# zcablii/RS_detection

Hardware: NVIDIA B200
Metric: tiles/s (Oriented R-CNN rotated-box hot path: RoIAlignRotated fwd + obb2poly + per-class nms_rotated) (higher is better)
Workload: dtype f32

## Files before the change

### rs_detection_b200/csrc/nms.cu

```cuda
#include <cub/device/device_radix_sort.cuh>
#include <cub/device/device_scan.cuh>
#include <cub/device/device_select.cuh>
#include <thrust/iterator/counting_iterator.h>

#include <mutex>
#include <vector>

#include "common.cuh"
#include "nms_engine.cuh"
#include "poly_iou.cuh"
#include "rotated_iou.cuh"

namespace rsdet {

constexpr int kNmsThreads = 128;
constexpr int kReduceThreads = 256;
constexpr size_t kCubTempBytes = 8u << 20;
constexpr int kFastSegs = 2048;

struct HBox { double x1, y1, x2, y2; };

template <int KIND> struct Traits;

template <> struct Traits<RSDET_NMS_ROTATED> {
    using Box = RBox; using Raw = float; using Thr = float;
    static constexpr int kRow = 5; static constexpr bool kScratch = true;
    __device__ static Box prep(const Raw* r) { return prep_rbox(r, 0); }
    static constexpr bool kRefine = true;
    __device__ static bool cheap(const Box& a, const Box& b) { return rbox_may_overlap(a, b); }
    __device__ static bool refine1(const Box& a, const Box& b, Thr thr) { return !rbox_iou_below(a, b, thr); }
    __device__ static bool refine2(const Box& a, const Box& b, Thr thr) { return !rbox_iou_below_strips(a, b, thr); }
    __device__ static bool suppress(const Box& a, const Box& b, Thr thr, float2* q) {
        return rotated_iou_pair<kNmsThreads>(a, b, q) > thr;
    }
};
template <> struct Traits<RSDET_NMS_ROTATED_GE> : Traits<RSDET_NMS_ROTATED> {
    __device__ static bool suppress(const Box& a, const Box& b, Thr thr, float2* q) {
        return rotated_iou_pair<kNmsThreads>(a, b, q) >= thr;
    }
};
template <> struct Traits<RSDET_NMS_POLY> {
    using Box = PolyBox; using Raw = float; using Thr = float;
    static constexpr int kRow = 8; static constexpr bool kScratch = true;
    __device__ static Box prep(const Raw* r) { return prep_polybox(r); }
    static constexpr bool kRefine = false;
    __device__ static bool cheap(const Box& a, const Box& b) { return !poly_pair_is_zero(a, b); }
    __device__ static bool refine1(const Box&, const Box&, Thr) { return true; }
    __device__ static bool refine2(const Box&, const Box&, Thr) { return true; }
    __device__ static bool suppress(const Box& a, const Box& b, Thr thr, float2* q) {
        return poly_iou_f32<kNmsThreads>(a, b, q) > thr;
    }
};
template <> struct Traits<RSDET_NMS_MERGE> {
    using Box = MBox; using Raw = double; using Thr = double;
    static constexpr int kRow = 8; static constexpr bool kScratch = false;
    __device__ static Box prep(const Raw* r) {
        Box b;
        double x1 = r[0], x2 = r[0], y1 = r[1], y2 = r[1];
        for (int i = 0; i < 4; i++) {
            b.p[2 * i] = r[2 * i]; b.p[2 * i + 1] = r[2 * i + 1];
            x1 = fmin(x1, r[2 * i]); x2 = fmax(x2, r[2 * i]);
            y1 = fmin(y1, r[2 * i + 1]); y2 = fmax(y2, r[2 * i + 1]);
        }
        b.x1 = x1; b.y1 = y1; b.x2 = x2; b.y2 = y2;
        return b;
    }
    static constexpr bool kRefine = false;
    __device__ static bool cheap(const Box& a, const Box& b) { return merge_hbb_overlap(a, b); }
    __device__ static bool refine1(const Box&, const Box&, Thr) { return true; }
    __device__ static bool refine2(const Box&, const Box&, Thr) { return true; }
    __device__ static bool suppress(const Box& a, const Box& b, Thr thr, float2*) { return !(iou_poly_d(a, b) <= thr); }
};
template <> struct Traits<RSDET_NMS_HBB> {
    using Box = HBox; using Raw = double; using Thr = double;
    static constexpr int kRow = 4; static constexpr bool kScratch = false;
    __device__ static Box prep(const Raw* r) { Box b; b.x1 = r[0]; b.y1 = r[1]; b.x2 = r[2]; b.y2 = r[3]; return b; }
    static constexpr bool kRefine = false;
    __device__ static bool cheap(const Box& a, const Box& b) {
        return (fmin(a.x2, b.x2) > fmax(a.x1, b.x1) && fmin(a.y2, b.y2) > fmax(a.y1, b.y1)) ||
               (a.x2 - a.x1) * (a.y2 - a.y1) + (b.x2 - b.x1) * (b.y2 - b.y1) == 0.0;
    }
    __device__ static bool refine1(const Box&, const Box&, Thr) { return true; }
// ... 540 lines not shown
    __shared__ int s_count3;
    const int tid = threadIdx.x, lane = tid & 31;
    const int T = (n + 63) >> 6;
    const int total = T * (T + 1) / 2;
    for (int u = blockIdx.x; u < total; u += gridDim.x) {
        if (only_flagged && !only_flagged[u]) continue;
        __syncthreads();
        int rb = (int)(((2.0 * T + 1.0) - sqrt((2.0 * T + 1.0) * (2.0 * T + 1.0) - 8.0 * (double)u)) * 0.5);
        rb = max(0, min(rb, T - 1));
        while (rb > 0 && rb * T - rb * (rb - 1) / 2 > u) rb--;
        while ((rb + 1) * T - (rb + 1) * rb / 2 <= u) rb++;
        const int cb = rb + (u - (rb * T - rb * (rb - 1) / 2));
        const int nr = min(64, n - rb * 64), nc = min(64, n - cb * 64);
        if (tid < 64) {
            float4 rc = make_float4(0.f, 0.f, -1e30f, 0.f);
            if (tid < nr) {
                const RBox bx = boxes[rb * 64 + tid];
                s_row[tid] = bx;
                rc = make_float4(bx.x, bx.y, bx.r, 0.f);
            }
            s_rowc[tid] = rc;
        } else if (tid - 64 < nc) {
            s_col[tid - 64] = boxes[cb * 64 + tid - 64];
        }
        __syncthreads();
        const bool diag = rb == cb;
        {
            const int c = tid & 63, rhalf = tid >> 6;
            unsigned hits = 0u;
            if (c < nc) {
                const float cx = s_col[c].x, cy = s_col[c].y, cr = s_col[c].r;
#pragma unroll 8
                for (int k = 0; k < 32; k++) {
                    const int r = 2 * k + rhalf;
                    const float4 rc = s_rowc[r];
                    const float rs = rc.z + cr, dx = rc.x - cx, dy = rc.y - cy;
                    const bool cand = (rs >= 0.f) && !(dx * dx + dy * dy > rs * rs) && (!diag || c > r);
                    hits |= (cand ? 1u : 0u) << k;
                }
            }
            const int mine = __popc(hits);
            int incl = mine;
#pragma unroll
            for (int o = 1; o < 32; o <<= 1) {
                const int y = __shfl_up_sync(0xffffffffu, incl, o);
                if (lane >= o) incl += y;
            }
            if (lane == 31) s_wsum[tid >> 5] = incl;
            __syncthreads();
            int pos = incl - mine;
            for (int w = 0; w < (tid >> 5); w++) pos += s_wsum[w];
            if (tid == kNmsThreads - 1) s_count = pos + mine;
            while (hits) {
                const int k = __ffs(hits) - 1;
                hits &= hits - 1;
                s_queue[pos++] = (unsigned short)(((2 * k + rhalf) << 6) | c);
            }
        }
        __syncthreads();
        const int cnt = s_count;
        for (int q0 = 0; q0 < cnt; q0 += kQ2) {
            const int n2 = compact_queue(s_queue + q0, min(kQ2, cnt - q0), s_queue2, &s_count2, s_wsum,
                                         [&](int p) { return !rbox_iou_below(s_row[p >> 6], s_col[p & 63], thr); });
            const int n3 = compact_queue(s_queue2, n2, s_queue3, &s_count3, s_wsum,
                                         [&](int p) { return !rbox_iou_below_strips(s_row[p >> 6], s_col[p & 63], thr); });
            for (int qi = tid; qi < n3; qi += kNmsThreads) {
                const int p = s_queue3[qi];
                const int r = p >> 6, c = p & 63;
                const int a = rb * 64 + r, b = cb * 64 + c;
                const float iou_ab = rotated_iou_pair<kNmsThreads>(s_row[r], s_col[c], s_pts + tid);
                const bool d_ab = GE ? iou_ab >= thr : iou_ab > thr;
                bool d_ba = d_ab;
                if (fabsf(iou_ab - thr) <= 1e-5f) {
                    const float iou_ba = rotated_iou_pair<kNmsThreads>(s_col[c], s_row[r], s_pts + tid);
                    d_ba = GE ? iou_ba >= thr : iou_ba > thr;
                }
                if (d_ab) atomicOr(&ov[(size_t)a * pitch + (b >> 6)], 1ull << (b & 63));
                if (d_ba) atomicOr(&ov[(size_t)b * pitch + (a >> 6)], 1ull << (a & 63));
            }
        }
    }
}

template <bool GE>
__global__ void __launch_bounds__(kNmsThreads, 8)
ov_filter_kernel(const RBox* __restrict__ boxes, int n, float thr, int2* __restrict__ pairs, unsigned int cap,
                 unsigned int* __restrict__ pair_count, uint8_t* __restrict__ tile_flags) {
    __shared__ RBox s_row[64];
    __shared__ RBox s_col[64];
    __shared__ unsigned short s_queue[64 * 64];
    constexpr int kQ2 = 1024;
    __shared__ unsigned short s_queue2[kQ2];
    __shared__ unsigned short s_queue3[kQ2];
    __shared__ unsigned int s_base;
    __shared__ float4 s_rowc[64];
    __shared__ int s_wsum[kNmsThreads / 32];
    __shared__ int s_count;
    __shared__ int s_count2;
    __shared__ int s_count3;
    const int tid = threadIdx.x, lane = tid & 31;
    const int T = (n + 63) >> 6;
    const int total = T * (T + 1) / 2;
    for (int u = blockIdx.x; u < total; u += gridDim.x) {
        __syncthreads();
        int rb = (int)(((2.0 * T + 1.0) - sqrt((2.0 * T + 1.0) * (2.0 * T + 1.0) - 8.0 * (double)u)) * 0.5);
        rb = max(0, min(rb, T - 1));
        while (rb > 0 && rb * T - rb * (rb - 1) / 2 > u) rb--;
        while ((rb + 1) * T - (rb + 1) * rb / 2 <= u) rb++;
        const int cb = rb + (u - (rb * T - rb * (rb - 1) / 2));
        const int nr = min(64, n - rb * 64), nc = min(64, n - cb * 64);
        if (tid < 64) {
            float4 rc = make_float4(0.f, 0.f, -1e30f, 0.f);
            if (tid < nr) {
                const RBox bx = boxes[rb * 64 + tid];
                s_row[tid] = bx;
                rc = make_float4(bx.x, bx.y, bx.r, 0.f);
            }
            s_rowc[tid] = rc;
        } else if (tid - 64 < nc) {
            s_col[tid - 64] = boxes[cb * 64 + tid - 64];
        }
        __syncthreads();
        const bool diag = rb == cb;
        {
            const int c = tid & 63, rhalf = tid >> 6;
            unsigned hits = 0u;
            if (c < nc) {
                const float cx = s_col[c].x, cy = s_col[c].y, cr = s_col[c].r;
#pragma unroll 8
                for (int k = 0; k < 32; k++) {
                    const int r = 2 * k + rhalf;
                    const float4 rc = s_rowc[r];
                    const float rs = rc.z + cr, dx = rc.x - cx, dy = rc.y - cy;
                    const bool cand = (rs >= 0.f) && !(dx * dx + dy * dy > rs * rs) && (!diag || c > r);
                    hits |= (cand ? 1u : 0u) << k;
                }
            }
            const int mine = __popc(hits);
            int incl = mine;
#pragma unroll
            for (int o = 1; o < 32; o <<= 1) {
                const int y = __shfl_up_sync(0xffffffffu, incl, o);
                if (lane >= o) incl += y;
            }
            if (lane == 31) s_wsum[tid >> 5] = incl;
            __syncthreads();
            int pos = incl - mine;
            for (int w = 0; w < (tid >> 5); w++) pos += s_wsum[w];
            if (tid == kNmsThreads - 1) s_count = pos + mine;
            while (hits) {
                const int k = __ffs(hits) - 1;
                hits &= hits - 1;
                s_queue[pos++] = (unsigned short)(((2 * k + rhalf) << 6) | c);
            }
        }
        __syncthreads();
        const int cnt = s_count;
        for (int q0 = 0; q0 < cnt; q0 += kQ2) {
            const int n2 = compact_queue(s_queue + q0, min(kQ2, cnt - q0), s_queue2, &s_count2, s_wsum,
                                         [&](int p) { return !rbox_iou_below(s_row[p >> 6], s_col[p & 63], thr); });
            const int n3 = compact_queue(s_queue2, n2, s_queue3, &s_count3, s_wsum,
                                         [&](int p) { return !rbox_iou_below_strips(s_row[p >> 6], s_col[p & 63], thr); });
            if (tid == 0) {
                const unsigned int base = n3 ? atomicAdd(pair_count, (unsigned int)n3) : 0u;
                if (n3 && base + (unsigned int)n3 > cap) { tile_flags[u] = 1; atomicAdd(pair_count + 1, 1u); }
                s_base = base;
            }
            __syncthreads();
            const unsigned int base = s_base;
            for (int qi = tid; qi < n3; qi += kNmsThreads) {
                if (base + (unsigned int)qi < cap) {
                    const int p = s_queue3[qi];
                    pairs[base + qi] = make_int2(rb * 64 + (p >> 6), cb * 64 + (p & 63));
                }
            }
            __syncthreads();
        }
    }
}

template <bool GE>
__global__ void __launch_bounds__(kNmsThreads, 8)
ov_clip_kernel(const RBox* __restrict__ boxes, const int2* __restrict__ pairs, unsigned int cap, const unsigned int* __restrict__ pair_count,
               float thr, unsigned long long* __restrict__ ov, int pitch) {
    __shared__ float2 s_pts[24 * kNmsThreads];
    const unsigned int count = min(*pair_count, cap);
    const int tid = threadIdx.x;
    for (unsigned int i = blockIdx.x * kNmsThreads + tid; i < count; i += gridDim.x * kNmsThreads) {
        const int2 pr = pairs[i];
        const RBox A = boxes[pr.x], B = boxes[pr.y];
        const float iou_ab = rotated_iou_pair<kNmsThreads>(A, B, s_pts + tid);
        const bool d_ab = GE ? iou_ab >= thr : iou_ab > thr;
        bool d_ba = d_ab;
        if (fabsf(iou_ab - thr) <= 1e-5f) {
            const float iou_ba = rotated_iou_pair<kNmsThreads>(B, A, s_pts + tid);
            d_ba = GE ? iou_ba >= thr : iou_ba > thr;
        }
        if (d_ab) atomicOr(&ov[(size_t)pr.x * pitch + (pr.y >> 6)], 1ull << (pr.y & 63));
        if (d_ba) atomicOr(&ov[(size_t)pr.y * pitch + (pr.x >> 6)], 1ull << (pr.x & 63));
    }
}

__global__ void __launch_bounds__(kReduceThreads, 1)
reduce_ov_kernel(SegTable tb, const int* __restrict__ idx_ls, int cand_per_box, const unsigned long long* __restrict__ ov,
                 int pitch, int n_boxes, uint8_t* __restrict__ keep_sorted) {
    extern __shared__ unsigned long long s_remv[];
    __shared__ int s_box2[2][64];
    __shared__ unsigned int s_diag32[128];
    __shared__ unsigned int s_rem32[2];
    __shared__ unsigned long long s_keep;
    const int tid = threadIdx.x, lane = tid & 31;
    const int nseg = tb.hdr[0];
    const int T = (n_boxes + 63) >> 6;
    for (int s = blockIdx.x; s < nseg; s += gridDim.x) {
        const int st = tb.seg_start[s];
        const int ns = tb.seg_start[s + 1] - st;
        const int nblk = (ns + 63) >> 6;
        __syncthreads();
        for (int j = tid; j < T; j += kReduceThreads) s_remv[j] = 0ull;
        for (int b = 0; b < nblk; b++) {
            const int nr = min(64, ns - b * 64);
            int* s_box = s_box2[b & 1];
            if (tid < 64) s_box[tid] = tid < nr ? idx_ls[st + b * 64 + tid] / cand_per_box : -1;
            __syncthreads();
            if (tid < 64) {
                const int a = s_box[tid];
                const bool rem = a < 0 || ((s_remv[a >> 6] >> (a & 63)) & 1ull);
                const unsigned m = __ballot_sync(0xffffffffu, rem);
                if (lane == 0) s_rem32[tid >> 5] = m;
            }
#pragma unroll 4
            for (int it = 0; it < 16; it++) {
                const int idx = it * kReduceThreads + tid;
                const int i = idx >> 6, j = idx & 63;
                bool bit = false;
                if (i < nr && j < nr && j > i) {
                    const int a = s_box[i], c = s_box[j];
                    bit = (ov[(size_t)a * pitch + (c >> 6)] >> (c & 63)) & 1ull;
                }
                const unsigned m = __ballot_sync(0xffffffffu, bit);
                if (lane == 0) s_diag32[idx >> 5] = m;
            }
            __syncthreads();
            if (tid == 0) {
                unsigned long long r = (unsigned long long)s_rem32[0] | ((unsigned long long)s_rem32[1] << 32), kb = 0ull;
#pragma unroll
                for (int i = 0; i < 64; i++) {
                    const bool alive = ((r >> i) & 1ull) == 0ull;
                    const unsigned long long d = (unsigned long long)s_diag32[2 * i] | ((unsigned long long)s_diag32[2 * i + 1] << 32);
                    kb |= alive ? (1ull << i) : 0ull;
                    r |= alive ? d : 0ull;
                }
                s_keep = kb;
            }
            __syncthreads();
            const unsigned long long kb = s_keep;
            if (tid < nr) keep_sorted[st + b * 64 + tid] = (uint8_t)((kb >> tid) & 1ull);
            if (kb && b + 1 < nblk) {
                const int jj = tid & 63, rg = tid >> 6;
// ... 635 lines not shown

constexpr int kMaxNmsBoxes = 1 << 18;

size_t nms_ws_bytes(int kind, int n, size_t mask_words) {
    size_t N = (size_t)(n > 0 ? n : 1);
    size_t b = 0;
    b += 2 * ws_bytes<unsigned long long>(N);
    b += 4 * ws_bytes<int>(N);
    b += 2 * ws_bytes<uint32_t>(N);
    b += align256(box_bytes(kind) * N);
    b += ws_bytes<int32_t>(N);
    b += ws_bytes<int>(64) + ws_bytes<int>(N + 2) + 2 * ws_bytes<long long>(N + 2) + ws_bytes<double>(N + 1);
    b += ws_bytes<unsigned long long>(mask_words ? mask_words : N * ((N + 63) / 64));
    b += 3 * ws_bytes<uint8_t>(N);
    b += 2 * ws_bytes<int64_t>(N);
    b += ws_bytes<int>(64) + ws_bytes<int>(kFastSegs);
    b += ws_bytes<unsigned long long>(2 * N / 64 + 8) + ws_bytes<int>(2 * N / 64 + 8);
    b += align256(kCubTempBytes + 16 * N);
    return b;
}

template <int KIND>
static void launch_kind(const NmsArgs& a, const int* idx, void* boxes, int32_t* label_sorted, SegTable tb,
                        unsigned long long* mask, cudaStream_t st, bool mask_phase, int* starts_unsorted, const int* gate = nullptr) {
    using Tr = Traits<KIND>;
    if (!mask_phase) {
        prep_sorted_kernel<KIND><<<ceil_div(a.n_max, 256), 256, 0, st>>>((const typename Tr::Raw*)a.dets, a.labels, idx, a.n_max,
                                                                        a.n_dev, (typename Tr::Box*)boxes, label_sorted,
                                                                        tb.hdr, starts_unsorted);
    } else {
        long long T = (a.n_max + 63) / 64;
        long long tiles = T * (T + 1) / 2;
        int grid = (int)(tiles < (long long)kNumSMs * 5 ? tiles : (long long)kNumSMs * 5);
        mask_tiles_kernel<KIND><<<grid, kNmsThreads, 0, st>>>((const typename Tr::Box*)boxes, tb, mask, gate);
    }
    count_launch();
}

static void dispatch_kind(const NmsArgs& a, const int* idx, void* boxes, int32_t* label_sorted, SegTable tb,
                          unsigned long long* mask, cudaStream_t st, bool mask_phase, int* starts_unsorted, const int* gate = nullptr) {
    switch (a.kind) {
        case RSDET_NMS_ROTATED: launch_kind<RSDET_NMS_ROTATED>(a, idx, boxes, label_sorted, tb, mask, st, mask_phase, starts_unsorted, gate); break;
        case RSDET_NMS_ROTATED_GE: launch_kind<RSDET_NMS_ROTATED_GE>(a, idx, boxes, label_sorted, tb, mask, st, mask_phase, starts_unsorted, gate); break;
        case RSDET_NMS_POLY: launch_kind<RSDET_NMS_POLY>(a, idx, boxes, label_sorted, tb, mask, st, mask_phase, starts_unsorted, gate); break;
        case RSDET_NMS_MERGE: launch_kind<RSDET_NMS_MERGE>(a, idx, boxes, label_sorted, tb, mask, st, mask_phase, starts_unsorted, gate); break;
        case RSDET_NMS_HBB_P1: launch_kind<RSDET_NMS_HBB_P1>(a, idx, boxes, label_sorted, tb, mask, st, mask_phase, starts_unsorted, gate); break;
        case RSDET_NMS_HBB_P1_F64: launch_kind<RSDET_NMS_HBB_P1_F64>(a, idx, boxes, label_sorted, tb, mask, st, mask_phase, starts_unsorted, gate); break;
        default: launch_kind<RSDET_NMS_HBB>(a, idx, boxes, label_sorted, tb, mask, st, mask_phase, starts_unsorted, gate); break;
    }
}

constexpr int kSparseMinRotated = 32768;

template <int KIND>
static void sp_launch_kind(int step, const void* boxes, SegTable tb, int n, const unsigned long long* key, const int* val,
                           const SparseWs& w, cudaStream_t st) {
    using Box = typename SpAdapt<KIND>::Box;
    const Box* b = (const Box*)boxes;
    switch (step) {
        case 0: sp_extent_kernel<KIND><<<ceil_div(n, 256), 256, 0, st>>>(b, tb, n, w); break;
        case 1: sp_keys_kernel<KIND><<<ceil_div(n + 1, 256), 256, 0, st>>>(b, tb, n, w); break;
        case 5: sp_estimate_kernel<KIND><<<ceil_div(n, 128), 128, 0, st>>>(b, tb, n, key, val, w); break;
        case 2: sp_sweep_kernel<KIND, false><<<ceil_div(n, 128), 128, 0, st>>>(b, tb, n, key, val, w); break;
        case 3: sp_sweep_kernel<KIND, true><<<ceil_div(n, 128), 128, 0, st>>>(b, tb, n, key, val, w); break;
        default: sp_iou_kernel<KIND><<<kNumSMs * 8, kNmsThreads, 0, st>>>(b, tb, n, w); break;
    }
}
static void sp_launch(int kind, int step, const void* boxes, SegTable tb, int n, const unsigned long long* key, const int* val,
                      const SparseWs& w, cudaStream_t st) {
    if (kind == RSDET_NMS_MERGE) sp_launch_kind<RSDET_NMS_MERGE>(step, boxes, tb, n, key, val, w, st);
    else if (kind == RSDET_NMS_ROTATED_GE) sp_launch_kind<RSDET_NMS_ROTATED_GE>(step, boxes, tb, n, key, val, w, st);
    else sp_launch_kind<RSDET_NMS_ROTATED>(step, boxes, tb, n, key, val, w, st);
}

static void launch_ov_matrix(const float* shared_boxes, int nb, float thr, bool ge, RBox* sb, unsigned long long* mask, size_t mask_cap,
                             int* cnt_scratch, cudaStream_t st) {
        const int Tov = (nb + 63) / 64;
        const int pitch = (Tov + 1) & ~1;
        prep_shared_kernel<<<ceil_div(nb, 256), 256, 0, st>>>(shared_boxes, nb, sb);
        cudaMemsetAsync(mask, 0, sizeof(unsigned long long) * (size_t)nb * pitch, st);
        long long tiles = (long long)Tov * (Tov + 1) / 2;
        int grid = (int)(tiles < (1ll << 22) ? tiles : (1ll << 22));
        const size_t used = (size_t)nb * pitch, flag_words = ((size_t)tiles + 7) / 8 + 1;
        const bool split = grid == tiles && mask_cap > used + flag_words + 4096;
        if (split) {
            uint8_t* tile_flags = (uint8_t*)(mask + used);
            int2* pairs = (int2*)(mask + used + flag_words);
            const size_t capz = mask_cap - used - flag_words;
            const unsigned int cap = (unsigned int)(capz < 0x7fffffffull ? capz : 0x7fffffffull);
            unsigned int* pair_count = (unsigned int*)(cnt_scratch + 32);
            cudaMemsetAsync(tile_flags, 0, flag_words * 8, st);
            cudaMemsetAsync(pair_count, 0, 2 * sizeof(int), st);
            const int cgrid = (int)(tiles < (long long)kNumSMs * 8 ? (long long)kNumSMs * 8 : (tiles < (long long)kNumSMs * 64 ? tiles : (long long)kNumSMs * 64));
            const int fgrid = (int)(tiles < (long long)kNumSMs * 2 ? tiles : (long long)kNumSMs * 2);
            if (ge) {
                ov_filter_kernel<true><<<grid, kNmsThreads, 0, st>>>(sb, nb, thr, pairs, cap, pair_count, tile_flags);
                ov_clip_kernel<true><<<cgrid, kNmsThreads, 0, st>>>(sb, pairs, cap, pair_count, thr, mask, pitch);
                ov_tiles_kernel<true><<<fgrid, kNmsThreads, 0, st>>>(sb, nb, thr, mask, pitch, tile_flags, pair_count + 1);
            } else {
                ov_filter_kernel<false><<<grid, kNmsThreads, 0, st>>>(sb, nb, thr, pairs, cap, pair_count, tile_flags);
                ov_clip_kernel<false><<<cgrid, kNmsThreads, 0, st>>>(sb, pairs, cap, pair_count, thr, mask, pitch);
                ov_tiles_kernel<false><<<fgrid, kNmsThreads, 0, st>>>(sb, nb, thr, mask, pitch, tile_flags, pair_count + 1);
            }
            count_launch(2);
        } else if (ge) {
            ov_tiles_kernel<true><<<grid, kNmsThreads, 0, st>>>(sb, nb, thr, mask, pitch, nullptr, nullptr);
        } else {
            ov_tiles_kernel<false><<<grid, kNmsThreads, 0, st>>>(sb, nb, thr, mask, pitch, nullptr, nullptr);
        }
}

static inline void allow_dyn_smem(const void* func, size_t bytes) {
    cudaFuncSetAttribute(func, cudaFuncAttributeMaxDynamicSharedMemorySize, (int)bytes);
}

int nms_run(const NmsArgs& a, void* workspace, size_t workspace_bytes, cudaStream_t st) {
    const int n = a.n_max;
    if (n < 0 || a.kind < 0 || a.kind > RSDET_NMS_HBB_P1_F64) return RSDET_EINVAL;
    if (n == 0) {
        if (a.num_keep) cudaMemsetAsync(a.num_keep, 0, sizeof(int32_t), st);
        return cuda_status();
    }
    if (!a.dets || !a.scores) return RSDET_EINVAL;
    if (n > (a.mask_words ? (1 << 20) : kMaxNmsBoxes)) return RSDET_ELIMIT;
    if (workspace_bytes < nms_ws_bytes(a.kind, n, a.mask_words)) return RSDET_EWORKSPACE;
    const bool f64 = a.kind == RSDET_NMS_MERGE || a.kind == RSDET_NMS_HBB || a.kind == RSDET_NMS_HBB_P1_F64;
    const size_t N = (size_t)n;

    Workspace ws(workspace, workspace_bytes);
    unsigned long long* keyA = ws.take<unsigned long long>(N);
    unsigned long long* keyB = ws.take<unsigned long long>(N);
    int* idxA = ws.take<int>(N);
    int* idxB = ws.take<int>(N);
    int* idxC = ws.take<int>(N);
    int* idxD = ws.take<int>(N);
    uint32_t* lkA = ws.take<uint32_t>(N);
    uint32_t* lkB = ws.take<uint32_t>(N);
    void* boxes = ws.take<char>(box_bytes(a.kind) * N);
    int32_t* label_sorted = ws.take<int32_t>(N);
    SegTable tb;
    tb.hdr = ws.take<int>(64);
    tb.seg_start = ws.take<int>(N + 2);
    tb.tile_pref = ws.take<long long>(N + 2);
    tb.mask_off = ws.take<long long>(N + 2);
    tb.seg_thr = ws.take<double>(N + 1);
    unsigned long long* mask = ws.take<unsigned long long>(a.mask_words ? a.mask_words : N * ((N + 63) / 64));
    uint8_t* keep_sorted = ws.take<uint8_t>(N);
    uint8_t* keep_tmp = ws.take<uint8_t>(N);
    uint8_t* flags = ws.take<uint8_t>(N);
    int64_t* vals = ws.take<int64_t>(N);
    int64_t* idx_scratch = ws.take<int64_t>(N);
    int* cnt_scratch = ws.take<int>(64);
    int* starts_unsorted = ws.take<int>(kFastSegs);
    unsigned long long* pub_keep = ws.take<unsigned long long>(2 * N / 64 + 8);
    int* pub_flag = ws.take<int>(2 * N / 64 + 8);
    size_t cub_bytes = kCubTempBytes + 16 * N;
    void* cub_tmp = ws.take<char>(cub_bytes);
    if (!ws.ok()) return RSDET_EWORKSPACE;

    const int* idx_score;
    if (f64) {
        make_keys_kernel<double, unsigned long long><<<ceil_div(n, 256), 256, 0, st>>>((const double*)a.scores, n, keyA, idxA, true);
        cub::DoubleBuffer<unsigned long long> dk(keyA, keyB);
        cub::DoubleBuffer<int> dv(idxA, idxB);
        size_t need = 0;
        cub::DeviceRadixSort::SortPairs(nullptr, need, dk, dv, n, 0, 64, st);
        if (need > cub_bytes) return RSDET_EWORKSPACE;
        cub::DeviceRadixSort::SortPairs(cub_tmp, need, dk, dv, n, 0, 64, st);
        idx_score = dv.Current();
    } else {
        uint32_t* kA = (uint32_t*)keyA;
        uint32_t* kB = (uint32_t*)keyB;
        make_keys_kernel<float, uint32_t><<<ceil_div(n, 256), 256, 0, st>>>((const float*)a.scores, n, kA, idxA, false);
        cub::DoubleBuffer<uint32_t> dk(kA, kB);
        cub::DoubleBuffer<int> dv(idxA, idxB);
        size_t need = 0;
        cub::DeviceRadixSort::SortPairs(nullptr, need, dk, dv, n, 0, 32, st);
        if (need > cub_bytes) return RSDET_EWORKSPACE;
        cub::DeviceRadixSort::SortPairs(cub_tmp, need, dk, dv, n, 0, 32, st);
        idx_score = dv.Current();
    }
    count_launch(4);
    const int* idx_ls = idx_score;
// ... 312 lines not shown
constexpr int kPipeThreads = 512;
constexpr int kMcFastMaxClasses = 4096;

__global__ void __launch_bounds__(1024)
mc_class_sort_kernel(const float* __restrict__ scores, const float* __restrict__ factors, int n, int C, float score_thr,
                     unsigned long long* __restrict__ skey, int* __restrict__ idx_ls, int* __restrict__ seg_count, SegTable tb) {
    extern __shared__ unsigned int s_k32[];
    __shared__ int s_warp_cnt[32], s_base;
    const int c = blockIdx.x, tid = threadIdx.x, lane = tid & 31, warp = tid >> 5;
    int Pmax = 64;
    while (Pmax < n) Pmax <<= 1;
    unsigned short* s_i16 = reinterpret_cast<unsigned short*>(s_k32 + Pmax);
    if (tid == 0) s_base = 0;
    __syncthreads();
    for (int i0 = 0; i0 < n; i0 += 1024) {
        const int i = i0 + tid;
        bool valid = false;
        float sc = 0.f;
        if (i < n) {
            sc = scores[(size_t)i * (C + 1) + c + 1];
            valid = sc > score_thr;
            if (valid && factors) sc = sc * factors[i];
        }
        const unsigned m = __ballot_sync(0xffffffffu, valid);
        if (lane == 0) s_warp_cnt[warp] = __popc(m);
        __syncthreads();
        int before = s_base;
        for (int w = 0; w < warp; w++) before += s_warp_cnt[w];
        if (valid) {
            const int pos = before + __popc(m & ((1u << lane) - 1u));
            s_k32[pos] = desc_key(sc);
            s_i16[pos] = (unsigned short)i;
        }
        __syncthreads();
        if (tid == 0) {
            int t = 0;
            for (int w = 0; w < 32; w++) t += s_warp_cnt[w];
            s_base += t;
        }
        __syncthreads();
    }
    const int cnt = s_base;
    int P = 2;
    while (P < cnt) P <<= 1;
    for (int q = cnt + tid; q < P; q += 1024) { s_k32[q] = 0xffffffffu; s_i16[q] = 0xffffu; }
    __syncthreads();
    const int chunk = P >= 2048 ? P >> 5 : 64, pairs = chunk >> 1, active_warps = P >= 64 ? P / chunk : 1;
    auto exchange = [&](int t, int j, int k) {
        const int i = ((t & ~(j - 1)) << 1) | (t & (j - 1)), l = i | j;
        const unsigned int ka = s_k32[i], kb = s_k32[l];
        const unsigned short ia = s_i16[i], ib = s_i16[l];
        const bool gt = ka > kb || (ka == kb && ia > ib);
        if (gt == ((i & k) == 0)) { s_k32[i] = kb; s_k32[l] = ka; s_i16[i] = ib; s_i16[l] = ia; }
    };
    for (int k = 2; k <= P; k <<= 1) {
        int j = k >> 1;
        if (j >= chunk) {
            __syncthreads();
            for (; j >= chunk; j >>= 1) {
                for (int t = tid; t < (P >> 1); t += 1024) exchange(t, j, k);
                __syncthreads();
            }
        }
        if (warp < active_warps)
            for (; j > 0; j >>= 1) {
                for (int u = lane; u < pairs && warp * pairs + u < (P >> 1); u += 32) exchange(warp * pairs + u, j, k);
                __syncwarp();
            }
    }
    __syncthreads();
    for (int q = tid; q < cnt; q += 1024) {
        const unsigned e = (unsigned)s_i16[q] * (unsigned)C + (unsigned)c;
        skey[(size_t)c * n + q] = ((unsigned long long)s_k32[q] << 32) | e;
        idx_ls[(size_t)c * n + q] = (int)e;
    }
    if (tid == 0) {
        seg_count[c] = cnt;
        tb.seg_start[c] = c * n;
        if (c == 0) tb.hdr[0] = C;
        if (c == C - 1) tb.seg_start[C] = C * n;
    }
}

__global__ void __launch_bounds__(256)
mc_fast_output_kernel(const float* __restrict__ bboxes, const float* __restrict__ scores, const float* __restrict__ factors, int n, int C,
                      const unsigned long long* __restrict__ skey, const int* __restrict__ seg_count, const int* __restrict__ kept_pos,
                      const int* __restrict__ keep_prefix, const int* __restrict__ kept_count, int max_num,
                      float* __restrict__ out_dets, int32_t* __restrict__ out_labels, int32_t* __restrict__ out_count) {
    const int lane = threadIdx.x & 31;
    const int cs = blockIdx.y, r = blockIdx.x * (blockDim.x >> 5) + (threadIdx.x >> 5);
    if (r >= kept_count[cs] && !(r == 0 && cs == 0)) return;
    int nk = 0;
    for (int c2 = lane; c2 < C; c2 += 32) nk += kept_count[c2];
    for (int o = 16; o > 0; o >>= 1) nk += __shfl_xor_sync(0xffffffffu, nk, o);
    int cnt = nk;
    if (nk > max_num) cnt = max_num >= 0 ? max_num : max(nk + max_num, 0);
    if (r == 0 && cs == 0 && lane == 0) *out_count = cnt;
    if (r >= kept_count[cs]) return;
    const int qs = kept_pos[(size_t)cs * n + r];
    const unsigned long long key = skey[(size_t)cs * n + qs];
    int rank = 0;
    for (int c2 = lane; c2 < C; c2 += 32) {
        if (c2 == cs) { rank += r; continue; }
        const unsigned long long* kk = skey + (size_t)c2 * n;
        const int len = seg_count[c2];
        int lo = 0, hi = len;
        while (lo < hi) {
            const int mid = (lo + hi) >> 1;
            if (kk[mid] < key) lo = mid + 1; else hi = mid;
        }
        rank += lo < len ? keep_prefix[(size_t)c2 * n + lo] : kept_count[c2];
    }
    for (int o = 16; o > 0; o >>= 1) rank += __shfl_xor_sync(0xffffffffu, rank, o);
    if (rank < cnt && lane < 7) {
        const int e = (int)(unsigned)(key & 0xffffffffull), i = e / C;
        if (lane < 5) out_dets[(size_t)rank * 6 + lane] = bboxes[(size_t)i * 5 + lane];
        else if (lane == 5) {
            float sc = scores[(size_t)i * (C + 1) + cs + 1];
            if (factors) sc = sc * factors[i];
            out_dets[(size_t)rank * 6 + 5] = sc;
        } else out_labels[rank] = cs;
    }
}

struct SideLane { cudaStream_t side; cudaEvent_t fork, join; };
static SideLane* side_lane(cudaStream_t user) {
    struct Key { int dev; cudaStream_t st; SideLane lane; };
    static std::vector<Key>* lanes = new std::vector<Key>();
    static std::mutex mu;
    int dev = 0;
    if (cudaGetDevice(&dev) != cudaSuccess) return nullptr;
    std::lock_guard<std::mutex> lk(mu);
    for (auto& k : *lanes)
        if (k.dev == dev && k.st == user) return &k.lane;
    if (lanes->size() >= 256) return nullptr;
    if (lanes->capacity() < 256) lanes->reserve(256);
    Key k;
    k.dev = dev; k.st = user;
    if (cudaStreamCreateWithFlags(&k.lane.side, cudaStreamNonBlocking) != cudaSuccess) { cudaGetLastError(); return nullptr; }
    if (cudaEventCreateWithFlags(&k.lane.fork, cudaEventDisableTiming) != cudaSuccess ||
        cudaEventCreateWithFlags(&k.lane.join, cudaEventDisableTiming) != cudaSuccess) { cudaGetLastError(); return nullptr; }
    lanes->push_back(k);
    return &lanes->back().lane;
}

static bool mc_fast_ok(int bbox_dim, int n, int C) {
    return bbox_dim == 5 && n >= 1 && n <= kMcFastMaxBoxes && C <= kMcFastMaxClasses;
}
static size_t mc_mask_words(int n, int num_classes);

static int mc_fast_run(const float* bboxes, const float* scores, int n, int C, float score_thr, float iou_thr, int max_num,
                       const float* factors, float* out_dets, int32_t* out_labels, int32_t* out_count, void* workspace,
                       size_t workspace_bytes, cudaStream_t st) {
    const size_t cap = (size_t)n * C;
    Workspace ws(workspace, workspace_bytes);
    unsigned long long* skey = ws.take<unsigned long long>(cap);
    int* idx_ls = ws.take<int>(cap);
    uint8_t* keep_sorted = ws.take<uint8_t>(cap);
    int* keep_prefix = ws.take<int>(cap);
    int* kept_pos = ws.take<int>(cap);
    int* seg_count = ws.take<int>(C);
    int* kept_count = ws.take<int>(C);
    int* cnt_scratch = ws.take<int>(64);
    SegTable tb;
    tb.hdr = ws.take<int>(64);
    tb.seg_start = ws.take<int>((size_t)C + 2);
    tb.tile_pref = nullptr; tb.mask_off = nullptr; tb.seg_thr = nullptr;
    RBox* sb = ws.take<RBox>(n);
    const size_t mask_cap = mc_mask_words(n, C);
    unsigned long long* mask = ws.take<unsigned long long>(mask_cap);
    if (!ws.ok()) return RSDET_EWORKSPACE;
    int P = 64;
    while (P < n) P <<= 1;
    const size_t sort_smem = (sizeof(unsigned int) + sizeof(unsigned short)) * (size_t)P;
    allow_dyn_smem((const void*)mc_class_sort_kernel, sort_smem);
    SideLane* sl = side_lane(st);
    if (sl && cudaEventRecord(sl->fork, st) == cudaSuccess && cudaStreamWaitEvent(sl->side, sl->fork, 0) == cudaSuccess) {
        mc_class_sort_kernel<<<C, 1024, sort_smem, sl->side>>>(scores, factors, n, C, score_thr, skey, idx_ls, seg_count, tb);
        cudaEventRecord(sl->join, sl->side);
    } else {
        cudaGetLastError();
        sl = nullptr;
        mc_class_sort_kernel<<<C, 1024, sort_smem, st>>>(scores, factors, n, C, score_thr, skey, idx_ls, seg_count, tb);
    }
    const int Tov = (n + 63) / 64, pitch = (Tov + 1) & ~1;
    launch_ov_matrix(bboxes, n, iou_thr, false, sb, mask, mask_cap, cnt_scratch, st);
    if (sl) cudaStreamWaitEvent(st, sl->join, 0);
    const size_t Ts = (size_t)(Tov | 1);
    const size_t piped = sizeof(unsigned long long) * (Ts + 3 * 64 * Ts) + sizeof(int) * (size_t)n;
    const size_t staged = sizeof(unsigned long long) * (5 * Ts + 2 * 64 * Ts) + sizeof(int) * (size_t)n;
    const int grid = C < kNumSMs ? C : kNumSMs;
    if (piped + 2048 <= 227 * 1024) {
        if (Tov <= 64) {
            allow_dyn_smem((const void*)reduce_ov_pipe_kernel<1, kPipeThreads>, piped);
            reduce_ov_pipe_kernel<1, kPipeThreads><<<grid, kPipeThreads, piped, st>>>(tb, idx_ls, C, mask, pitch, n, keep_sorted, seg_count, keep_prefix,
                                                                         kept_count, kept_pos);
        } else {
            allow_dyn_smem((const void*)reduce_ov_pipe_kernel<2, kPipeThreads>, piped);
            reduce_ov_pipe_kernel<2, kPipeThreads><<<grid, kPipeThreads, piped, st>>>(tb, idx_ls, C, mask, pitch, n, keep_sorted, seg_count, keep_prefix,
                                                                         kept_count, kept_pos);
        }
    } else {
        allow_dyn_smem((const void*)reduce_ov_staged_kernel<2, false>, 200 * 1024);
        reduce_ov_staged_kernel<2, false><<<grid, kReduceThreads, staged, st>>>(tb, idx_ls, C, mask, pitch, n, keep_sorted, nullptr, seg_count,
                                                                              keep_prefix, kept_count, kept_pos);
    }
    mc_fast_output_kernel<<<dim3((unsigned)((n + 7) / 8), (unsigned)C), 256, 0, st>>>(bboxes, scores, factors, n, C, skey, seg_count, kept_pos,
                                                                                     keep_prefix, kept_count, max_num, out_dets, out_labels,
                                                                                     out_count);
    count_launch(8);
    return cuda_status();
}

static size_t mc_mask_words(int n, int num_classes) {
    size_t N = (size_t)(n > 0 ? n : 1);
    return (size_t)(num_classes > 0 ? num_classes : 1) * N * ((N + 63) / 64 + 1);
}

extern "C" size_t rsdet_multiclass_nms_rotated_workspace_bytes(int n, int num_classes) {
    size_t cap = (size_t)(n > 0 ? n : 1) * (size_t)(num_classes > 0 ? num_classes : 1);
    if (cap > (1u << 20) || n > kMaxNmsBoxes) return 0;
    return ws_bytes<float>(cap * 5) + ws_bytes<float>(cap) + ws_bytes<int32_t>(cap) + ws_bytes<int>(64) +
           ws_bytes<int64_t>(cap) + ws_bytes<int32_t>(64) + ws_bytes<int>(kMcHist) +
           nms_ws_bytes(RSDET_NMS_ROTATED, (int)cap, mc_mask_words(n, num_classes));
}

extern "C" int rsdet_multiclass_nms_rotated(const float* multi_bboxes, int bbox_dim, const float* multi_scores, int n,
                                            int num_classes, float score_thr, float iou_thr, int max_num,
                                            const float* score_factors, float* out_dets, int32_t* out_labels,
                                            int32_t* out_count, void* workspace, size_t workspace_bytes, void* stream) {
    if (n < 0 || num_classes <= 0 || !out_count) return RSDET_EINVAL;
    if (bbox_dim != 5 && bbox_dim != 5 * (num_classes + 1)) return RSDET_EINVAL;
    cudaStream_t st = (cudaStream_t)stream;
    if (n == 0) {
        cudaMemsetAsync(out_count, 0, sizeof(int32_t), st);
        return cuda_status();
    }
    if (!multi_bboxes || !multi_scores || !out_dets || !out_labels) return RSDET_EINVAL;
    long long capll = (long long)n * num_classes;
    if (capll > (1 << 20) || n > kMaxNmsBoxes) return RSDET_ELIMIT;
    int cap = (int)capll;
    if (workspace_bytes < rsdet_multiclass_nms_rotated_workspace_bytes(n, num_classes)) return RSDET_EWORKSPACE;
    if (mc_fast_ok(bbox_dim, n, num_classes))
        return mc_fast_run(multi_bboxes, multi_scores, n, num_classes, score_thr, iou_thr, max_num, score_factors, out_dets, out_labels,
                           out_count, workspace, workspace_bytes, st);
    Workspace ws(workspace, workspace_bytes);
    float* cbox = ws.take<float>((size_t)cap * 5);
    float* cscore = ws.take<float>(cap);
    int32_t* clabel = ws.take<int32_t>(cap);
    int* n_valid = ws.take<int>(64);
    int64_t* kidx = ws.take<int64_t>(cap);
    int32_t* nkeep = ws.take<int32_t>(64);
    int* class_counts = ws.take<int>(kMcHist);
    void* sub = ws.base + ws.used;
    size_t sub_bytes = workspace_bytes - ws.used;
    const bool use_counts = bbox_dim == 5 && num_classes <= kMcHist;
    cudaMemsetAsync(n_valid, 0, sizeof(int), st);
    if (use_counts) cudaMemsetAsync(class_counts, 0, sizeof(int) * num_classes, st);
    mc_expand_kernel<<<ceil_div(cap, 256), 256, 0, st>>>(multi_bboxes, bbox_dim, multi_scores, n, num_classes, score_thr,
                                                        score_factors, cbox, cscore, clabel, n_valid,
                                                        use_counts ? class_counts : nullptr);
    count_launch();
    NmsArgs a{RSDET_NMS_ROTATED, cbox, cscore, clabel, cap, n_valid, (double)iou_thr, nullptr, 0, nullptr, nullptr, kidx, nkeep};
    a.mask_words = mc_mask_words(n, num_classes);
    a.label_bits = 1;
    while ((1 << a.label_bits) - 1 < num_classes) a.label_bits++;
    if (bbox_dim == 5) {
        a.shared_boxes = multi_bboxes;
        a.n_shared = n;
        a.cand_per_box = num_classes;
        if (use_counts) { a.class_counts = class_counts; a.num_classes = num_classes; }
    }
    int rc = nms_run(a, sub, sub_bytes, st);
    if (rc != RSDET_OK) return rc;
    mc_output_kernel<<<ceil_div(cap, 256), 256, 0, st>>>(kidx, nkeep, max_num, cbox, cscore, clabel, out_dets, out_labels,
                                                        out_count, cap);
    count_launch();
    return cuda_status();
}
```

Baseline: 5686.

## Prefetch column tiles asynchronously in overlap filter and compact multiclass output launch

The overlap filter kernel now processes runs of two triangular tiles per block. It reuses the loaded row tile and prefetches the next column tile into a double buffer with cp.async, so global load latency can hide behind candidate compaction. The multiclass output kernel changes from a grid of n×C mostly idle warps to a capped grid. A per-block prefix sum over kept counts sends warps only to kept detections. Costs: each block repeats the prefix over C classes, the split path is now enabled for more grid sizes, and each filter block does serial work over two tiles.

```diff
diff --git a/rs_detection_b200/csrc/nms.cu b/rs_detection_b200/csrc/nms.cu
--- a/rs_detection_b200/csrc/nms.cu
+++ b/rs_detection_b200/csrc/nms.cu
@@ -1,3 +1,4 @@
+#include <cuda_pipeline.h>
 #include <cub/device/device_radix_sort.cuh>
 #include <cub/device/device_scan.cuh>
 #include <cub/device/device_select.cuh>
@@ -704,12 +705,24 @@
     }
 }
 
+__device__ __forceinline__ void ov_prefetch_cols(const RBox* __restrict__ boxes, int n, int cb, RBox* s_col) {
+    const int c = threadIdx.x - 64;
+    if (c >= 0 && c < min(64, n - cb * 64)) {
+        const float4* src = reinterpret_cast<const float4*>(boxes + cb * 64 + c);
+        float4* dst = reinterpret_cast<float4*>(s_col + c);
+#pragma unroll
+        for (int k = 0; k < (int)(sizeof(RBox) / sizeof(float4)); k++) __pipeline_memcpy_async(dst + k, src + k, sizeof(float4));
+    }
+    __pipeline_commit();
+}
+
+constexpr int kFilterRun = 2;
 template <bool GE>
 __global__ void __launch_bounds__(kNmsThreads, 8)
 ov_filter_kernel(const RBox* __restrict__ boxes, int n, float thr, int2* __restrict__ pairs, unsigned int cap,
                  unsigned int* __restrict__ pair_count, uint8_t* __restrict__ tile_flags) {
     __shared__ RBox s_row[64];
-    __shared__ RBox s_col[64];
+    __shared__ RBox s_cols[2][64];
     __shared__ unsigned short s_queue[64 * 64];
     constexpr int kQ2 = 1024;
     __shared__ unsigned short s_queue2[kQ2];
@@ -723,15 +736,18 @@
     const int tid = threadIdx.x, lane = tid & 31;
     const int T = (n + 63) >> 6;
     const int total = T * (T + 1) / 2;
-    for (int u = blockIdx.x; u < total; u += gridDim.x) {
-        __syncthreads();
-        int rb = (int)(((2.0 * T + 1.0) - sqrt((2.0 * T + 1.0) * (2.0 * T + 1.0) - 8.0 * (double)u)) * 0.5);
+    for (int u0 = blockIdx.x * kFilterRun; u0 < total; u0 += gridDim.x * kFilterRun) {
+        const int u1 = min(u0 + kFilterRun, total);
+        __syncthreads();
+        int rb = (int)(((2.0 * T + 1.0) - sqrt((2.0 * T + 1.0) * (2.0 * T + 1.0) - 8.0 * (double)u0)) * 0.5);
         rb = max(0, min(rb, T - 1));
-        while (rb > 0 && rb * T - rb * (rb - 1) / 2 > u) rb--;
-        while ((rb + 1) * T - (rb + 1) * rb / 2 <= u) rb++;
-        const int cb = rb + (u - (rb * T - rb * (rb - 1) / 2));
-        const int nr = min(64, n - rb * 64), nc = min(64, n - cb * 64);
-        if (tid < 64) {
+        while (rb > 0 && rb * T - rb * (rb - 1) / 2 > u0) rb--;
+        while ((rb + 1) * T - (rb + 1) * rb / 2 <= u0) rb++;
+        int cb = rb + (u0 - (rb * T - rb * (rb - 1) / 2));
+        ov_prefetch_cols(boxes, n, cb, s_cols[0]);
+        for (int u = u0, loaded_rb = -1; u < u1; u++) {
+        if (rb != loaded_rb && tid < 64) {
+            const int nr = min(64, n - rb * 64);
             float4 rc = make_float4(0.f, 0.f, -1e30f, 0.f);
             if (tid < nr) {
                 const RBox bx = boxes[rb * 64 + tid];
@@ -739,64 +755,70 @@
                 rc = make_float4(bx.x, bx.y, bx.r, 0.f);
             }
             s_rowc[tid] = rc;
-        } else if (tid - 64 < nc) {
-            s_col[tid - 64] = boxes[cb * 64 + tid - 64];
-        }
-        __syncthreads();
+        }
+        loaded_rb = rb;
+        __pipeline_wait_prior(0);
+        __syncthreads();
+        const RBox* s_col = s_cols[(u - u0) & 1];
+        const int nc = min(64, n - cb * 64);
         const bool diag = rb == cb;
-        {
-            const int c = tid & 63, rhalf = tid >> 6;
-            unsigned hits = 0u;
-            if (c < nc) {
-                const float cx = s_col[c].x, cy = s_col[c].y, cr = s_col[c].r;
+        const int rb_u = rb, cb_u = cb;
+        if (++cb == T) cb = ++rb;
+        if (u + 1 < u1) ov_prefetch_cols(boxes, n, cb, s_cols[(u + 1 - u0) & 1]);
+            {
+                const int c = tid & 63, rhalf = tid >> 6;
+                unsigned hits = 0u;
+                if (c < nc) {
+                    const float cx = s_col[c].x, cy = s_col[c].y, cr = s_col[c].r;
 #pragma unroll 8
-                for (int k = 0; k < 32; k++) {
-                    const int r = 2 * k + rhalf;
-                    const float4 rc = s_rowc[r];
-                    const float rs = rc.z + cr, dx = rc.x - cx, dy = rc.y - cy;
-                    const bool cand = (rs >= 0.f) && !(dx * dx + dy * dy > rs * rs) && (!diag || c > r);
-                    hits |= (cand ? 1u : 0u) << k;
-                }
-            }
-            const int mine = __popc(hits);
-            int incl = mine;
-#pragma unroll
-            for (int o = 1; o < 32; o <<= 1) {
-                const int y = __shfl_up_sync(0xffffffffu, incl, o);
-                if (lane >= o) incl += y;
-            }
-            if (lane == 31) s_wsum[tid >> 5] = incl;
+                    for (int k = 0; k < 32; k++) {
+                        const int r = 2 * k + rhalf;
+                        const float4 rc = s_rowc[r];
+                        const float rs = rc.z + cr, dx = rc.x - cx, dy = rc.y - cy;
+                        const bool cand = (rs >= 0.f) && !(dx * dx + dy * dy > rs * rs) && (!diag || c > r);
+                        hits |= (cand ? 1u : 0u) << k;
+                    }
+                }
+                const int mine = __popc(hits);
+                int incl = mine;
+#pragma unroll
+                for (int o = 1; o < 32; o <<= 1) {
+                    const int y = __shfl_up_sync(0xffffffffu, incl, o);
+                    if (lane >= o) incl += y;
+                }
+                if (lane == 31) s_wsum[tid >> 5] = incl;
+                __syncthreads();
+                int pos = incl - mine;
+                for (int w = 0; w < (tid >> 5); w++) pos += s_wsum[w];
+                if (tid == kNmsThreads - 1) s_count = pos + mine;
+                while (hits) {
+                    const int k = __ffs(hits) - 1;
+                    hits &= hits - 1;
+                    s_queue[pos++] = (unsigned short)(((2 * k + rhalf) << 6) | c);
+                }
+            }
             __syncthreads();
-            int pos = incl - mine;
-            for (int w = 0; w < (tid >> 5); w++) pos += s_wsum[w];
-            if (tid == kNmsThreads - 1) s_count = pos + mine;
-            while (hits) {
-                const int k = __ffs(hits) - 1;
-                hits &= hits - 1;
-                s_queue[pos++] = (unsigned short)(((2 * k + rhalf) << 6) | c);
-            }
-        }
-        __syncthreads();
-        const int cnt = s_count;
-        for (int q0 = 0; q0 < cnt; q0 += kQ2) {
-            const int n2 = compact_queue(s_queue + q0, min(kQ2, cnt - q0), s_queue2, &s_count2, s_wsum,
-                                         [&](int p) { return !rbox_iou_below(s_row[p >> 6], s_col[p & 63], thr); });
-            const int n3 = compact_queue(s_queue2, n2, s_queue3, &s_count3, s_wsum,
-                                         [&](int p) { return !rbox_iou_below_strips(s_row[p >> 6], s_col[p & 63], thr); });
-            if (tid == 0) {
-                const unsigned int base = n3 ? atomicAdd(pair_count, (unsigned int)n3) : 0u;
-                if (n3 && base + (unsigned int)n3 > cap) { tile_flags[u] = 1; atomicAdd(pair_count + 1, 1u); }
-                s_base = base;
-            }
-            __syncthreads();
-            const unsigned int base = s_base;
-            for (int qi = tid; qi < n3; qi += kNmsThreads) {
-                if (base + (unsigned int)qi < cap) {
-                    const int p = s_queue3[qi];
-                    pairs[base + qi] = make_int2(rb * 64 + (p >> 6), cb * 64 + (p & 63));
-                }
-            }
-            __syncthreads();
+            const int cnt = s_count;
+            for (int q0 = 0; q0 < cnt; q0 += kQ2) {
+                const int n2 = compact_queue(s_queue + q0, min(kQ2, cnt - q0), s_queue2, &s_count2, s_wsum,
+                                             [&](int p) { return !rbox_iou_below(s_row[p >> 6], s_col[p & 63], thr); });
+                const int n3 = compact_queue(s_queue2, n2, s_queue3, &s_count3, s_wsum,
+                                             [&](int p) { return !rbox_iou_below_strips(s_row[p >> 6], s_col[p & 63], thr); });
+                if (tid == 0) {
+                    const unsigned int base = n3 ? atomicAdd(pair_count, (unsigned int)n3) : 0u;
+                    if (n3 && base + (unsigned int)n3 > cap) { tile_flags[u] = 1; atomicAdd(pair_count + 1, 1u); }
+                    s_base = base;
+                }
+                __syncthreads();
+                const unsigned int base = s_base;
+                for (int qi = tid; qi < n3; qi += kNmsThreads) {
+                    if (base + (unsigned int)qi < cap) {
+                        const int p = s_queue3[qi];
+                        pairs[base + qi] = make_int2(rb_u * 64 + (p >> 6), cb_u * 64 + (p & 63));
+                    }
+                }
+                __syncthreads();
+            }
         }
     }
 }
@@ -1598,7 +1620,7 @@
         long long tiles = (long long)Tov * (Tov + 1) / 2;
         int grid = (int)(tiles < (1ll << 22) ? tiles : (1ll << 22));
         const size_t used = (size_t)nb * pitch, flag_words = ((size_t)tiles + 7) / 8 + 1;
-        const bool split = grid == tiles && mask_cap > used + flag_words + 4096;
+        const bool split = tiles <= (1ll << 22) && mask_cap > used + flag_words + 4096;
         if (split) {
             uint8_t* tile_flags = (uint8_t*)(mask + used);
             int2* pairs = (int2*)(mask + used + flag_words);
@@ -1609,12 +1631,13 @@
             cudaMemsetAsync(pair_count, 0, 2 * sizeof(int), st);
             const int cgrid = (int)(tiles < (long long)kNumSMs * 8 ? (long long)kNumSMs * 8 : (tiles < (long long)kNumSMs * 64 ? tiles : (long long)kNumSMs * 64));
             const int fgrid = (int)(tiles < (long long)kNumSMs * 2 ? tiles : (long long)kNumSMs * 2);
+            const int rgrid = (int)((tiles + kFilterRun - 1) / kFilterRun);
             if (ge) {
-                ov_filter_kernel<true><<<grid, kNmsThreads, 0, st>>>(sb, nb, thr, pairs, cap, pair_count, tile_flags);
+                ov_filter_kernel<true><<<rgrid, kNmsThreads, 0, st>>>(sb, nb, thr, pairs, cap, pair_count, tile_flags);
                 ov_clip_kernel<true><<<cgrid, kNmsThreads, 0, st>>>(sb, pairs, cap, pair_count, thr, mask, pitch);
                 ov_tiles_kernel<true><<<fgrid, kNmsThreads, 0, st>>>(sb, nb, thr, mask, pitch, tile_flags, pair_count + 1);
             } else {
-                ov_filter_kernel<false><<<grid, kNmsThreads, 0, st>>>(sb, nb, thr, pairs, cap, pair_count, tile_flags);
+                ov_filter_kernel<false><<<rgrid, kNmsThreads, 0, st>>>(sb, nb, thr, pairs, cap, pair_count, tile_flags);
                 ov_clip_kernel<false><<<cgrid, kNmsThreads, 0, st>>>(sb, pairs, cap, pair_count, thr, mask, pitch);
                 ov_tiles_kernel<false><<<fgrid, kNmsThreads, 0, st>>>(sb, nb, thr, mask, pitch, tile_flags, pair_count + 1);
             }
@@ -2093,44 +2116,67 @@
     }
 }
 
-__global__ void __launch_bounds__(256)
+constexpr int kMcOutThreads = 256;
+__global__ void __launch_bounds__(kMcOutThreads)
 mc_fast_output_kernel(const float* __restrict__ bboxes, const float* __restrict__ scores, const float* __restrict__ factors, int n, int C,
                       const unsigned long long* __restrict__ skey, const int* __restrict__ seg_count, const int* __restrict__ kept_pos,
                       const int* __restrict__ keep_prefix, const int* __restrict__ kept_count, int max_num,
                       float* __restrict__ out_dets, int32_t* __restrict__ out_labels, int32_t* __restrict__ out_count) {
-    const int lane = threadIdx.x & 31;
-    const int cs = blockIdx.y, r = blockIdx.x * (blockDim.x >> 5) + (threadIdx.x >> 5);
-    if (r >= kept_count[cs] && !(r == 0 && cs == 0)) return;
-    int nk = 0;
-    for (int c2 = lane; c2 < C; c2 += 32) nk += kept_count[c2];
-    for (int o = 16; o > 0; o >>= 1) nk += __shfl_xor_sync(0xffffffffu, nk, o);
+    extern __shared__ int s_first[];
+    __shared__ int s_wsum[kMcOutThreads / 32];
+    const int tid = threadIdx.x, lane = tid & 31, warp = tid >> 5;
+    {
+        const int per = (C + kMcOutThreads - 1) / kMcOutThreads, c0 = min(tid * per, C), c1 = min(c0 + per, C);
+        int mine = 0;
+        for (int c2 = c0; c2 < c1; c2++) mine += kept_count[c2];
+        int incl = mine;
+        for (int o = 1; o < 32; o <<= 1) {
+            const int y = __shfl_up_sync(0xffffffffu, incl, o);
+            if (lane >= o) incl += y;
+        }
+        if (lane == 31) s_wsum[warp] = incl;
+        __syncthreads();
+        int run = incl - mine;
+        for (int w = 0; w < warp; w++) run += s_wsum[w];
+        for (int c2 = c0; c2 < c1; c2++) { s_first[c2] = run; run += kept_count[c2]; }
+        if (tid == kMcOutThreads - 1) s_first[C] = run;
+        __syncthreads();
+    }
+    const int nk = s_first[C];
     int cnt = nk;
     if (nk > max_num) cnt = max_num >= 0 ? max_num : max(nk + max_num, 0);
-    if (r == 0 && cs == 0 && lane == 0) *out_count = cnt;
-    if (r >= kept_count[cs]) return;
-    const int qs = kept_pos[(size_t)cs * n + r];
-    const unsigned long long key = skey[(size_t)cs * n + qs];
-    int rank = 0;
-    for (int c2 = lane; c2 < C; c2 += 32) {
-        if (c2 == cs) { rank += r; continue; }
-        const unsigned long long* kk = skey + (size_t)c2 * n;
-        const int len = seg_count[c2];
-        int lo = 0, hi = len;
-        while (lo < hi) {
-            const int mid = (lo + hi) >> 1;
-            if (kk[mid] < key) lo = mid + 1; else hi = mid;
-        }
-        rank += lo < len ? keep_prefix[(size_t)c2 * n + lo] : kept_count[c2];
-    }
-    for (int o = 16; o > 0; o >>= 1) rank += __shfl_xor_sync(0xffffffffu, rank, o);
-    if (rank < cnt && lane < 7) {
-        const int e = (int)(unsigned)(key & 0xffffffffull), i = e / C;
-        if (lane < 5) out_dets[(size_t)rank * 6 + lane] = bboxes[(size_t)i * 5 + lane];
-        else if (lane == 5) {
-            float sc = scores[(size_t)i * (C + 1) + cs + 1];
-            if (factors) sc = sc * factors[i];
-            out_dets[(size_t)rank * 6 + 5] = sc;
-        } else out_labels[rank] = cs;
+    if (blockIdx.x == 0 && tid == 0) *out_count = cnt;
+    for (int f = blockIdx.x * (kMcOutThreads / 32) + warp; f < nk; f += gridDim.x * (kMcOutThreads / 32)) {
+        int lo_c = 0, hi_c = C;
+        while (hi_c - lo_c > 1) {
+            const int mid = (lo_c + hi_c) >> 1;
+            if (s_first[mid] <= f) lo_c = mid; else hi_c = mid;
+        }
+        const int cs = lo_c, r = f - s_first[cs];
+        const int qs = kept_pos[(size_t)cs * n + r];
+        const unsigned long long key = skey[(size_t)cs * n + qs];
+        int rank = 0;
+        for (int c2 = lane; c2 < C; c2 += 32) {
+            if (c2 == cs) { rank += r; continue; }
+            const unsigned long long* kk = skey + (size_t)c2 * n;
+            const int len = seg_count[c2];
+            int lo = 0, hi = len;
+            while (lo < hi) {
+                const int mid = (lo + hi) >> 1;
+                if (kk[mid] < key) lo = mid + 1; else hi = mid;
+            }
+            rank += lo < len ? keep_prefix[(size_t)c2 * n + lo] : kept_count[c2];
+        }
+        for (int o = 16; o > 0; o >>= 1) rank += __shfl_xor_sync(0xffffffffu, rank, o);
+        if (rank < cnt && lane < 7) {
+            const int e = (int)(unsigned)(key & 0xffffffffull), i = e / C;
+            if (lane < 5) out_dets[(size_t)rank * 6 + lane] = bboxes[(size_t)i * 5 + lane];
+            else if (lane == 5) {
+                float sc = scores[(size_t)i * (C + 1) + cs + 1];
+                if (factors) sc = sc * factors[i];
+                out_dets[(size_t)rank * 6 + 5] = sc;
+            } else out_labels[rank] = cs;
+        }
     }
 }
 
@@ -2216,9 +2262,11 @@
         reduce_ov_staged_kernel<2, false><<<grid, kReduceThreads, staged, st>>>(tb, idx_ls, C, mask, pitch, n, keep_sorted, nullptr, seg_count,
                                                                               keep_prefix, kept_count, kept_pos);
     }
-    mc_fast_output_kernel<<<dim3((unsigned)((n + 7) / 8), (unsigned)C), 256, 0, st>>>(bboxes, scores, factors, n, C, skey, seg_count, kept_pos,
-                                                                                     keep_prefix, kept_count, max_num, out_dets, out_labels,
-                                                                                     out_count);
+    const long long out_ctas = ((long long)n * C + kMcOutThreads / 32 - 1) / (kMcOutThreads / 32);
+    const int ogrid = (int)(out_ctas < kNumSMs * 8 ? out_ctas : kNumSMs * 8);
+    mc_fast_output_kernel<<<ogrid, kMcOutThreads, sizeof(int) * ((size_t)C + 1), st>>>(bboxes, scores, factors, n, C, skey, seg_count,
+                                                                                        kept_pos, keep_prefix, kept_count, max_num,
+                                                                                        out_dets, out_labels, out_count);
     count_launch(8);
     return cuda_status();
 }
```

Result: no change. 5706 (median of 6 runs) (+0.4%).
